# knelk/enerf

Measured on AMD Instinct MI355X. Metric: train_rays_per_sec, higher is better.
Workload: dtype f32

## Files before the change

### enerf_amd/_lib.py

```python
import ctypes
import os

_HERE = os.path.dirname(os.path.abspath(__file__))
LIB_PATH = os.path.join(_HERE, "lib", "libenerf_hip.so")
if os.environ.get("ENERF_LIB_PATH"):
    LIB_PATH = os.environ["ENERF_LIB_PATH"]

_c = ctypes
_vp, _u32, _f32, _int, _sz = _c.c_void_p, _c.c_uint32, _c.c_float, _c.c_int, _c.c_size_t

SIGNATURES = {
    "enerf_near_far_from_aabb": [_vp, _vp, _vp, _u32, _f32, _vp, _vp, _vp],
    "enerf_polar_from_ray": [_vp, _vp, _f32, _u32, _vp, _vp],
    "enerf_morton3D": [_vp, _u32, _vp, _vp],
    "enerf_morton3D_invert": [_vp, _u32, _vp, _vp],
    "enerf_packbits": [_vp, _u32, _f32, _vp, _vp],
    "enerf_march_rays_train": [_vp, _vp, _vp, _f32, _f32, _u32, _u32, _u32, _u32, _u32, _vp, _vp, _vp, _vp, _vp,
                               _vp, _vp, _u32, _vp],
    "enerf_march_fuse_near_far": [_vp, _f32],
    "enerf_march_mirror_count": [_vp],
    "enerf_march_rays_train_ex": [_vp, _vp, _vp, _f32, _f32, _u32, _u32, _u32, _u32, _u32, _vp, _vp, _vp, _vp, _vp,
                                  _vp, _vp, _u32, _u32, _vp],
    "enerf_march_rays_train_count": [_vp, _vp, _vp, _f32, _f32, _u32, _u32, _u32, _u32, _vp, _vp, _vp, _vp, _u32, _u32,
                                     _vp],
# ... 33 lines not shown
    "enerf_grid_encode_backward_ex": [_vp, _vp, _vp, _vp, _vp, _u32, _u32, _u32, _u32, _f32, _u32, _int, _vp, _vp,
                                   _u32, _int, _int, _f32, _f32, _u32, _u32, _vp],
    "enerf_grid_records_discard": [_vp],
    "enerf_mlp32_signal_next_reduce": [_int],
    "enerf_stream_wait_mlp32_signal": [_vp],
    "enerf_debug_workspace_ordering": [_int],
    "enerf_mlp32_valid_rows": [_vp],
    "enerf_mlp32_valid_rows_ex": [_vp, _u32, _u32],
    "enerf_mlp32_io16": [_int],
    "enerf_grid_adam_from_records_ex": [_vp, _vp, _vp, _vp, _vp, _u32, _u32, _f32, _f32, _f32, _f32, _u32, _u32, _vp, _vp,
                                        _vp, _vp, _vp, _vp, _vp, _vp],
    "enerf_grid_adam_from_records": [_vp, _vp, _vp, _vp, _vp, _u32, _u32, _f32, _f32, _f32, _f32, _u32, _vp],
    "enerf_sh_encode_forward": [_vp, _vp, _u32, _u32, _u32, _int, _vp, _int, _vp],
    "enerf_sh_encode_backward": [_vp, _vp, _u32, _u32, _u32, _vp, _vp, _int, _vp],
    "enerf_ffmlp_forward": [_vp, _vp, _u32, _u32, _u32, _u32, _u32, _u32, _u32, _vp, _vp, _int, _vp],
    "enerf_ffmlp_inference": [_vp, _vp, _u32, _u32, _u32, _u32, _u32, _u32, _u32, _vp, _vp, _int, _vp],
    "enerf_ffmlp_backward": [_vp, _vp, _vp, _vp, _u32, _u32, _u32, _u32, _u32, _u32, _u32, _int, _vp, _vp, _vp,
                             _int, _vp],
    "enerf_ffnerf_inference": [_vp, _vp, _vp, _vp, _u32, _int, _vp, _vp, _vp],
    "enerf_mlp32_forward": [_vp, _vp, _u32, _u32, _u32, _u32, _u32, _u32, _vp, _vp, _u32, _u32, _vp, _vp],
    "enerf_mlp32_forward_p": [_vp, _vp, _u32, _u32, _u32, _u32, _u32, _u32, _u32, _u32, _vp, _vp, _u32, _u32, _vp, _vp,
                              _vp],
    "enerf_mlp32_backward_p": [_vp, _vp, _vp, _vp, _u32, _u32, _u32, _vp, _u32, _u32, _u32, _u32, _u32, _vp, _vp, _u32,
                               _u32, _vp, _u32, _vp, _vp, _u32, _vp],
    "enerf_mlp32_forward_sh": [_vp, _vp, _u32, _u32, _u32, _u32, _u32, _u32, _vp, _vp, _u32, _u32, _vp, _vp, _vp],
    "enerf_mlp32_backward": [_vp, _vp, _vp, _vp, _u32, _u32, _u32, _u32, _u32, _vp, _vp, _vp, _u32, _u32, _vp, _u32, _vp, _vp,
                             _u32, _vp],
    "enerf_sh_encode_forward_strided": [_vp, _vp, _u32, _u32, _u32, _vp],
    "enerf_debug_grid_level_mask": [_u32],
    "enerf_debug_sweep_route": [_u32, _u32],
    "enerf_debug_sweep_schedule": [_u32, _u32, _u32, _vp, _u32],
    "enerf_debug_mlp32_wgrad_blocks": [_u32],
    "enerf_debug_mlp32_grid_caps": [_u32, _u32],
    "enerf_debug_march_wave_max_rays": [_u32],
    "enerf_debug_march_bg_blocks": [_u32],
    "enerf_debug_march_clip": [_int],
    "enerf_march_rays_use_box": [_int],
    "enerf_grid_owner_range": [ctypes.c_uint64, ctypes.c_uint64, _f32],
    "enerf_ffmlp_recompute": [_int],
    "enerf_amp_begin": [_vp, _vp, _vp, _vp],
    "enerf_amp_end": [_f32, _f32, _int, _vp],
    "enerf_amp_cancel": [],
    "enerf_debug_march_thread_min_rays": [_u32],
    "enerf_event_loss_fwd_bwd": [_vp, _vp, _vp, _u32, _u32, _u32, _f32, _f32, _f32, _vp, _vp, _vp, _vp, _vp],
    "enerf_event_loss_fwd_bwd_c": [_vp, _vp, _vp, _u32, _u32, _u32, _f32, _f32, _f32, _vp, _vp, _vp, _vp, _u32, _vp],
    "enerf_event_pair_rays": [_vp, _vp, _vp, _vp, _u32, _vp, _vp, _u32, _u32, _vp, _vp, _vp, _vp, _u32, _f32, _f32, _f32,
                              _f32, _vp, _vp, _vp, _vp, _vp, _vp, _vp, _vp, _vp],
    "enerf_event_single_pair_rays": [_vp, _u32, _vp, _vp, _u32, _vp, _vp, _u32, _vp, _vp, _vp, _vp, _u32, _f32, _f32, _f32,
                                     _f32, _vp, _vp, _vp, _vp, _vp, _vp, _vp, _vp, _vp, _vp],
    "enerf_no_event_rays": [_vp, _u32, _vp, _vp, _u32, _c.c_double, _c.c_double, _vp, _vp, _vp, _vp, _u32, _f32, _f32,
                            _f32, _f32, _vp, _vp, _vp, _vp, _vp, _vp, _vp, _vp],
    "enerf_occupied_box_update": [_vp, _u32, _u32, _f32, _vp],
    "enerf_debug_mlp32_fused_backward": [_int],
    "enerf_mlp32_precision": [_int],
    "enerf_mlp32_recompute": [_int],
    "enerf_debug_grid_bwd_binned": [_u32, _u32],
    "enerf_density_grid_cells": [_vp, _u32, _u32, _f32, _u32, _c.c_uint64, _vp, _vp, _vp],
    "enerf_mark_untrained_grid": [_vp, _u32, _u32, _f32, _f32, _f32, _f32, _u32, _u32, _f32, _vp, _vp],
    "enerf_density_grid_update": [_vp, _vp, _u32, _u32, _u32, _f32, _f32, _f32, _vp, _vp, _vp, _u32, _vp, _vp],
    "enerf_adam_step": [_vp, _vp, _vp, _vp, _sz, _f32, _f32, _f32, _f32, _u32, _int, _vp],
    "enerf_allocate_splitk": [_sz],
    "enerf_free_splitk": [],
    "enerf_mlp32_defer_reduce": [_int],
    "enerf_march_train_samples": [_c.POINTER(_c.c_uint64), _int, _vp],
    "enerf_prof_enable": [_int],
    "enerf_prof_reset": [],
# ... 207 lines not shown
```

### enerf_amd/csrc/mlp32.hip

```cpp
#include <hip/hip_runtime.h>
#include <cstdlib>
#include <cstring>
#include <hip/hip_ext.h>

#include "common.h"
#include "mlp32_common.h"
#include "sh_basis.h"

using namespace enerf;
using namespace enerf_mlp32;

namespace {


#ifdef ENERF_MLP_TIMING
__device__ unsigned long long g_mlp_phase[16];
#define MLP_PH(k)                                                  \
    do {                                                           \
        const unsigned long long t_ = __builtin_amdgcn_s_memtime(); \
        ph[k] += t_ - t_last;                                      \
        t_last = t_;                                               \
    } while (0)
#else
#define MLP_PH(k)
// ... 736 lines not shown
}

__global__ void __launch_bounds__(1024) k_mlp32_reduce_w2(ReduceJob a, ReduceJob b, uint32_t* found_inf) {
    const uint32_t na = (a.NW + 63u) / 64u;
    if (blockIdx.x < na) reduce_w_body(a.partial, a.nblocks, a.NW, a.dst, blockIdx.x, found_inf, a.stride);
    else reduce_w_body(b.partial, b.nblocks, b.NW, b.dst, blockIdx.x - na, found_inf, b.stride);
}

static ValidRows g_valid = {nullptr, 0, 0};
static bool g_signal_armed = false;
static bool g_signal_recorded = false;
static hipEvent_t g_signal_event = nullptr;
#ifndef ENERF_SIGNAL_SYSTEM_RELEASE
constexpr unsigned kSignalEventFlags = hipEventDisableTiming | hipEventReleaseToDevice;
#else
constexpr unsigned kSignalEventFlags = hipEventDisableTiming;
#endif
hipEvent_t signal_event() {
    if (!g_signal_event && hipEventCreateWithFlags(&g_signal_event, kSignalEventFlags) != hipSuccess) g_signal_event = nullptr;
    return g_signal_event;
}
static bool g_defer_next = false;
static DeferredReduce g_pending = {};

bool g_fused_bwd = true;
int g_precision = 1;
inline bool ops16(int mode) { return mode == 2 || mode == 3; }
bool g_io16_p = false;
bool g_recompute = true;
inline bool recompute_for(uint32_t num_hidden) { return g_recompute || num_hidden == 3; }
uint32_t g_wgrad_blocks = 0;

uint32_t g_fwd_blocks = 0;
uint32_t g_bwd_blocks = 0;

bool split_bwd_shape(int mode, uint32_t num_hidden, uint32_t out_dim, uint32_t x_layout) {
    return g_fused_bwd && mode != 0 && out_dim <= 16 &&
           (num_hidden <= 2 || (ops16(mode) && num_hidden == 3 && x_layout == 0));
}

uint32_t pgrid(uint32_t B, uint32_t cap) {
    const uint32_t blocks = div_up(div_up(B, 32), 4);
    return blocks < cap ? blocks : cap;
}

}

extern "C" {

int enerf_mlp32_valid_rows(const int32_t* device_count) { return enerf_mlp32_valid_rows_ex(device_count, 0, 0); }
int enerf_mlp32_valid_rows_ex(const int32_t* device_count, uint32_t base, uint32_t cap) {
    g_valid = {device_count, device_count ? base : 0, device_count ? cap : 0};
    return 0;
}

int enerf_mlp32_io16(int on) {
    const int prev = g_io16_p ? 1 : 0;
    if (on >= 0) g_io16_p = on != 0;
    return prev;
}

int enerf_mlp32_precision(int mode) {
    const int prev = g_precision;
    if (mode >= 0 && mode <= 3) g_precision = mode;
    return prev;
}

int enerf_mlp32_recompute(int on) {
    const int prev = g_recompute ? 1 : 0;
    if (on >= 0) g_recompute = on != 0;
    return prev;
}

int enerf_debug_mlp32_fused_backward(int on) {
    g_fused_bwd = on != 0;
    return 0;
}

int enerf_debug_mlp32_grid_caps(uint32_t fwd_blocks, uint32_t bwd_blocks) {
    g_fwd_blocks = fwd_blocks;
    g_bwd_blocks = bwd_blocks;
    return 0;
}

int enerf_debug_mlp32_wgrad_blocks(uint32_t blocks) {
    g_wgrad_blocks = blocks;
    return 0;
}

}


static WSrc seg_src(const float* const* wseg, uint32_t num_hidden, uint32_t w0_cols, uint32_t nerf_perm, const ValidRows& rows) {
    WSrc w;
    for (uint32_t k = 0; k < 4; k++) w.seg[k] = (k == 0 || k == 3 || k < num_hidden) ? wseg[k] : nullptr;
    w.w0_cols = w0_cols;
    w.nerf_perm = nerf_perm;
    w.valid_rows = rows.count;
    w.valid_base = rows.base;
    w.valid_cap = rows.cap;
    return w;
}
static WDst seg_dst(float* const* dwseg, uint32_t num_hidden, uint32_t w0_cols, uint32_t nerf_perm, uint32_t overwrite) {
    WDst d;
    for (uint32_t k = 0; k < 4; k++) d.seg[k] = (k == 0 || k == 3 || k < num_hidden) ? dwseg[k] : nullptr;
    d.w0_cols = w0_cols;
    d.nerf_perm = nerf_perm;
    d.overwrite = overwrite;
    return d;
}
static WSrc blob_src(const float* W, uint32_t num_hidden, const ValidRows& rows) {
    const float* seg[4] = {W, W + HID * IN, W + HID * IN + HID * HID, W + HID * IN + (num_hidden - 1) * HID * HID};
    return seg_src(seg, num_hidden, IN, 0, rows);
}
static WDst blob_dst(float* dW, uint32_t num_hidden, uint32_t overwrite) {
// ... 6 lines not shown
        return ENERF_E_BADARG;
    }
    if ((nerf_perm && w0_cols != 31 && w0_cols != IN) || (!nerf_perm && w0_cols != IN)) {
        set_error("%s: first-layer rows are 32 floats, or 31 / 32 with the NeRF colour permutation", what);
        return ENERF_E_BADARG;
    }
    return 0;
}

static int mlp32_forward_impl(const float* X, WSrc W, uint32_t B, uint32_t in_dim, uint32_t out_dim,
                              uint32_t num_hidden, uint32_t activation, uint32_t output_activation, float* fb, float* Y,
                              uint32_t x_layout, uint32_t y_stride, float* y0_exp, const float* sh_dirs,
                              enerf_stream_t stream, int mode, bool io16) {
    if (B == 0) return 0;
    if (sh_dirs && !((num_hidden == 1 || (num_hidden == 2 && mode != 0)) && x_layout == 1 && Y && out_dim <= 16 &&
                     (y_stride == 0 ? out_dim : y_stride) >= 32))
        ENERF_BADARG("mlp32_forward_sh: needs one hidden layer (two in the bf16 modes), level-major input, out_dim <= 16 "
                     "and rows of >= 32 floats");
    if (in_dim != IN) ENERF_BADARG("mlp32: in_dim must be 32 (pad the input), got %u", in_dim);
    if (out_dim == 0 || out_dim > 32) ENERF_BADARG("mlp32: out_dim must be in [1, 32], got %u", out_dim);
    if (num_hidden < 1 || num_hidden > 3) ENERF_BADARG("mlp32: num_hidden must be 1..3, got %u", num_hidden);
    if (activation != 0 && activation != 6) ENERF_BADARG("mlp32: activation must be relu (0) or none (6)");
    if (x_layout > 1) ENERF_BADARG("mlp32: x_layout must be 0 (row-major) or 1 (level-major), got %u", x_layout);
    if (output_activation != 0 && output_activation != 3 && output_activation != 6)
        ENERF_BADARG("mlp32: output activation must be relu (0), sigmoid (3) or none (6)");
    if (y_stride == 0) y_stride = out_dim;
    if (y_stride < out_dim) ENERF_BADARG("mlp32: y_stride %u < out_dim %u", y_stride, out_dim);
    if (int eg = single_device_guard("mlp32_forward")) return eg;
    hipStream_t s = (hipStream_t)stream;
    ProfScope prof(ENERF_K_FFMLP_FWD, s, mode != 0);
    prof.units((double)B);
    const bool sigma_only_shape = num_hidden == 1 && !fb && !Y && y0_exp && x_layout == 1;
    const bool lds_operands = mode == 1 && !sigma_only_shape;
    const uint32_t grid = pgrid(B, g_fwd_blocks ? g_fwd_blocks : (lds_operands ? 768 : 512));
    size_t lds = sizeof(float) * (HID * IN + (num_hidden - 1) * HID * HID + out_dim * HID);
    if (lds_operands && lds < (size_t)(8 + 8 * (num_hidden - 1)) * 2048) lds = (size_t)(8 + 8 * (num_hidden - 1)) * 2048;
#define MLP32_FWD2(NHV, TR, XLV) \
    k_mlp32_fwd<NHV, TR, XLV><<<grid, 256, lds, s>>>(X, W, fb, Y, B, out_dim, activation, output_activation, y_stride, y0_exp)
#define MLP32_FWD(NHV)                                        \
    do {                                                      \
        if (fb) {                                             \
            if (x_layout == 0) MLP32_FWD2(NHV, true, 0);      \
            else MLP32_FWD2(NHV, true, 1);                    \
        } else {                                              \
            if (x_layout == 0) MLP32_FWD2(NHV, false, 0);     \
            else MLP32_FWD2(NHV, false, 1);                   \
        }                                                     \
    } while (0)
    const bool sigma_only = num_hidden == 1 && !fb && !Y && y0_exp && x_layout == 1;
    if (mode != 0) {
        const bool store_fb = fb != nullptr && !(recompute_for(num_hidden) && split_bwd_shape(mode, num_hidden, out_dim, x_layout));
        (mode == 3 ? mlp32s_f16_launch_fwd : mlp32s_launch_fwd)(
            mode == 1 ? 3 : 1, num_hidden, store_fb, x_layout, sigma_only, X, W, fb, Y, B, out_dim, activation,
            output_activation, y_stride, y0_exp, sh_dirs, grid, lds, s, prof.start(), prof.stop(), io16);
    } else if (sh_dirs) {
        const ShNorm4 nrm = make_sh_norm4();
        if (fb)
            k_mlp32_fwd<1, true, 1, false, true><<<grid, 256, lds, s>>>(X, W, fb, Y, B, out_dim, activation,
                                                                        output_activation, y_stride, y0_exp, sh_dirs, nrm);
        else
            k_mlp32_fwd<1, false, 1, false, true><<<grid, 256, lds, s>>>(X, W, fb, Y, B, out_dim, activation,
                                                                         output_activation, y_stride, y0_exp, sh_dirs, nrm);
    } else if (sigma_only)
        k_mlp32_fwd<1, false, 1, true><<<grid, 256, lds, s>>>(X, W, fb, Y, B, out_dim, activation, output_activation,
                                                              y_stride, y0_exp);
    else if (num_hidden == 1) MLP32_FWD(1);
    else if (num_hidden == 2) MLP32_FWD(2);
    else MLP32_FWD(3);
#undef MLP32_FWD
#undef MLP32_FWD2
    ENERF_LAUNCH_CHECK("mlp32_forward");
    return 0;
}

int enerf::mlp32_forward_p(const float* X, const float* const* wseg, uint32_t w0_cols, uint32_t nerf_perm, uint32_t B,
                           uint32_t in_dim, uint32_t out_dim, uint32_t num_hidden, uint32_t activation,
                           uint32_t output_activation, float* fb, float* Y, uint32_t x_layout, uint32_t y_stride,
                           float* y0_exp, const float* sh_dirs, enerf_stream_t stream, const MlpCall& c) {
    if (num_hidden < 1 || num_hidden > 3) ENERF_BADARG("mlp32: num_hidden must be 1..3, got %u", num_hidden);
    if (int e = segs_ok((const void* const*)wseg, num_hidden, w0_cols, nerf_perm, "mlp32_forward_p")) return e;
    if (c.io16 && c.mode != 3) ENERF_BADARG("mlp32_forward_p: 16-bit I/O (enerf_mlp32_io16) serves precision 3 only");
    if (c.io16 && (num_hidden < 2 || out_dim > 16 || x_layout != 0 || sh_dirs || y0_exp || !Y))
        ENERF_BADARG("mlp32_forward_p: 16-bit I/O needs two or three hidden layers, out_dim <= 16, row-major X, an output "
                     "Y and no SH / density epilogue");
    return mlp32_forward_impl(X, seg_src(wseg, num_hidden, w0_cols, nerf_perm, c.rows), B, in_dim, out_dim, num_hidden,
                              activation, output_activation, fb, Y, x_layout, y_stride, y0_exp, sh_dirs, stream, c.mode, c.io16);
}

static int mlp32_backward_impl(const float* dY, const float* X, WSrc W, const float* fb, uint32_t B, uint32_t in_dim,
                               uint32_t out_dim, uint32_t num_hidden, uint32_t activation, float* bb, float* dX,
                               WDst dW, uint32_t x_layout, uint32_t dy_stride, const float* y_sigmoid,
                               uint32_t y_sigmoid_stride, const float* dsigma, const float* h0, uint32_t h0_stride,
                               enerf_stream_t stream, int mode, bool io16, bool signal, hipEvent_t* signalled,
                               DeferredReduce* pair) {
    if (B == 0) return 0;
    if (in_dim != IN) ENERF_BADARG("mlp32: in_dim must be 32, got %u", in_dim);
// ... 482 lines not shown
```

### enerf_amd/csrc/mlp32_common.h

```cpp
#pragma once
#include <hip/hip_runtime.h>

#include "common.h"
#include "sh_basis.h"

namespace enerf_mlp32 {
using namespace enerf;

typedef float f32x16 __attribute__((ext_vector_type(16)));
constexpr int HID = 64;
constexpr int IN = 32;

__device__ __forceinline__ f32x16 mma(float a, float b, f32x16 c) {
    return __builtin_amdgcn_mfma_f32_32x32x2f32(a, b, c, 0, 0, 0);
}
__device__ __forceinline__ int nrow(int q, int h) { return (q & 3) + 8 * (q >> 2) + 4 * h; }

__device__ __forceinline__ float act_fwd(float x, uint32_t a) { return a == 0 ? (x > 0 ? x : 0.0f) : x; }
__device__ __forceinline__ float out_act_fwd(float x, uint32_t a) {
    return a == 0 ? (x > 0 ? x : 0.0f) : (a == 3 ? 1.0f / (1.0f + expf(-x)) : x);
}

struct DySource {
    const float* dY;
// ... 157 lines not shown
__device__ __forceinline__ float fb_at(const float* tilebase, int srow, int n) {
    return tilebase[(n >> 5) * 1024 + ((n >> 3) & 3) * 256 + (srow + 32 * ((n >> 2) & 1)) * 4 + (n & 3)];
}

template <int XL>
__device__ __forceinline__ int kmap(int p, int h) {
    return XL == 0 ? 16 * h + p : 4 * (p >> 1) + 2 * h + (p & 1);
}

template <int XL>
__device__ __forceinline__ void load_x(const float* __restrict__ X, uint32_t tile, int j, int h, uint32_t B, uint32_t Bp,
                                       float (&x)[16]) {
    const size_t s = (size_t)tile * 32 + j;
    const bool valid = s < B;
    if (XL == 0) {
        const size_t sc = valid ? s : (size_t)B - 1;
#pragma unroll
        for (int v = 0; v < 4; v++) {
            const float4 t = *reinterpret_cast<const float4*>(X + sc * IN + 16 * h + 4 * v);
            x[4 * v] = t.x; x[4 * v + 1] = t.y; x[4 * v + 2] = t.z; x[4 * v + 3] = t.w;
        }
    } else {
#pragma unroll
        for (int q = 0; q < 8; q++) {
            const float2 t = *reinterpret_cast<const float2*>(X + ((size_t)(2 * q + h) * Bp + s) * 2);
            x[2 * q] = t.x; x[2 * q + 1] = t.y;
        }
    }
    if (!valid) {
#pragma unroll
        for (int p = 0; p < 16; p++) x[p] = 0.0f;
    }
}

void mlp32s_launch_fwd(int prec, uint32_t num_hidden, bool train, uint32_t x_layout, bool sigma_only, const float* X, const WSrc& W,
                       float* fb, float* Y, uint32_t B, uint32_t out_dim, uint32_t act, uint32_t out_act,
                       uint32_t y_stride, float* y0_exp, const float* sh_dirs, uint32_t grid, size_t lds, hipStream_t s,
                       hipEvent_t ev_start = nullptr, hipEvent_t ev_stop = nullptr, bool io16 = false);
void mlp32s_launch_bwd(int prec, uint32_t num_hidden, uint32_t x_layout, const DySource& dys, const float* X, const WSrc& W,
                       const float* fb, float* dX, float* partial, uint32_t B, uint32_t out_dim, uint32_t act,
                       uint32_t grid, hipStream_t s, hipEvent_t ev_start = nullptr, hipEvent_t ev_stop = nullptr,
                       bool recompute = false, bool io16 = false);

void mlp32s_f16_launch_fwd(int prec, uint32_t num_hidden, bool train, uint32_t x_layout, bool sigma_only, const float* X,
                           const WSrc& W, float* fb, float* Y, uint32_t B, uint32_t out_dim, uint32_t act, uint32_t out_act,
                           uint32_t y_stride, float* y0_exp, const float* sh_dirs, uint32_t grid, size_t lds, hipStream_t s,
                           hipEvent_t ev_start = nullptr, hipEvent_t ev_stop = nullptr, bool io16 = false);
void mlp32s_f16_launch_bwd(int prec, uint32_t num_hidden, uint32_t x_layout, const DySource& dys, const float* X,
                           const WSrc& W, const float* fb, float* dX, float* partial, uint32_t B, uint32_t out_dim,
                           uint32_t act, uint32_t grid, hipStream_t s, hipEvent_t ev_start = nullptr,
                           hipEvent_t ev_stop = nullptr, bool recompute = false, bool io16 = false);

constexpr uint32_t kNerfFragBytes = 44 * 2048;
constexpr uint32_t kNerfMapBytes = 44 * 512 * 4;
constexpr uint32_t kNerfPartMapBytes = ((HID * IN + 16 * HID) + (HID * IN + HID * HID + 16 * HID)) * 4;
constexpr uint32_t kNerfWsBytes = kNerfFragBytes + kNerfMapBytes + kNerfPartMapBytes;
constexpr uint32_t kNerfPartialStride = (HID * IN + 16 * HID) + (HID * IN + HID * HID + 16 * HID);
constexpr uint32_t kNerfSigmaWords = HID * IN + 16 * HID;
#ifndef NERF_FWD_ONE_PER_CU
constexpr uint32_t kNerfFwdPerCu = 3;
#else
constexpr uint32_t kNerfFwdPerCu = 1;
#endif
void nerf_launch_frags(const float* ws0, const float* ws1, const float* wc0, const float* wc1, const float* wc2,
                       uint32_t w0_cols, uint32_t out_c, uint32_t* frags, hipStream_t s);
void nerf_launch_frag_map(uint32_t w0_cols, uint32_t out_c, uint32_t* map, hipStream_t s);
void nerf_launch_fwd(const float* X, const float* dirs, const uint32_t* frags, float* sigma, float* rgb, uint32_t B,
                     uint32_t out_c, const int32_t* valid_rows, uint32_t valid_base, uint32_t valid_cap, uint32_t grid,
                     hipStream_t s, hipEvent_t ev_start = nullptr, hipEvent_t ev_stop = nullptr);
void nerf_launch_bwd(const float* X, const float* dirs, const float* g_rgb, const float* rgb, const float* g_sigma,
                     float sigma_scale, const uint32_t* frags, float* dX, float* partial, uint32_t B, uint32_t out_c,
                     const int32_t* valid_rows, uint32_t valid_base, uint32_t valid_cap, uint32_t grid, hipStream_t s,
                     hipEvent_t ev_start = nullptr, hipEvent_t ev_stop = nullptr);

int ffmlp16_forward(int dtype, const void* X, const float* W32, uint32_t B, uint32_t num_hidden, uint32_t activation,
                    void* Y, hipStream_t s);
int ffmlp16_backward(int dtype, const void* dY, const void* X, const float* W32, uint32_t B, uint32_t num_hidden,
// ... 4 lines not shown
```

### enerf_amd/csrc/mlp32s.hip

```cpp
#include <hip/hip_runtime.h>
#include <hip/hip_ext.h>

#include "mlp32_common.h"
#include "mlp32s_ops.h"

namespace enerf_mlp32 {


__device__ __forceinline__ void load_x16(const void* __restrict__ X, uint32_t tile, int j, int h, uint32_t B, bf16x8 (&f)[2]) {
    const size_t s = (size_t)tile * 32 + j;
    const bool valid = s < B;
    const size_t sc = valid ? s : (size_t)B - 1;
    const uint4* p = reinterpret_cast<const uint4*>(reinterpret_cast<const elem16*>(X) + sc * IN + 16 * h);
    uint4 a = p[0], b = p[1];
    if (!valid) a = b = make_uint4(0u, 0u, 0u, 0u);
    f[0] = __builtin_bit_cast(bf16x8, a);
    f[1] = __builtin_bit_cast(bf16x8, b);
}
__device__ __forceinline__ void store4_16(void* base, size_t elem, float a, float b, float c, float d) {
    typedef elem16 e4 __attribute__((ext_vector_type(4)));
    const e4 v = {(elem16)a, (elem16)b, (elem16)c, (elem16)d};
    *reinterpret_cast<e4*>(reinterpret_cast<elem16*>(base) + elem) = v;
}

constexpr bool fwd_weights_in_lds(bool SIG, int P) { return P == 3 && !SIG; }
typedef unsigned u32x4w __attribute__((ext_vector_type(4)));

#ifdef ENERF_MLP32S_F16
#define k_mlp32s_fwd k_mlp32h_fwd
#define k_mlp32s_bwd k_mlp32h_bwd
#define k_mlp32s_mark k_mlp32h_mark
#endif
template <int NH, bool TRAIN, int XL, bool SIG = false, bool SH = false, int P = 3, bool IO16 = false>
__global__ void __launch_bounds__(256, fwd_weights_in_lds(SIG, P) ? 3 : 1) k_mlp32s_fwd(const float* __restrict__ X, WSrc W,
                                                    float* __restrict__ fb, float* __restrict__ Y, uint32_t B,
                                                    uint32_t out_dim, uint32_t act, uint32_t out_act, uint32_t y_stride,
                                                    float* __restrict__ y0_exp, const float* __restrict__ sh_dirs = nullptr,
                                                    ShNorm4 nrm = ShNorm4{}) {
    extern __shared__ __attribute__((aligned(16))) float wl[];
    const int lane = lane_id(), j = lane & 31, h = lane >> 5;
    const uint32_t Bp = (B + 31u) & ~31u;
    static_assert(!IO16 || (P == 1 && XL == 0 && !SIG && !SH && !TRAIN), "16-bit I/O: bf16 / fp16 operands, row-major, plain");
    float x[16];
    bf16x8 xraw[2];
    {
        const uint32_t tile0 = blockIdx.x * (blockDim.x >> 6) + (threadIdx.x >> 6);
        if (tile0 < Bp / 32) {
            if constexpr (IO16) load_x16(X, tile0, j, h, B, xraw);
            else load_x<XL>(X, tile0, j, h, B, Bp, x);
        }
    }
    stage_rot(wl, W, NH, out_dim);

    typedef FragT<P> Frag;
    constexpr bool WL = fwd_weights_in_lds(SIG, P);
    Frag w0[2][2], wh[NH > 1 ? NH - 1 : 1][2][2][2], wo[2][2];
    float wsig[2][16];
#pragma unroll
    for (int ob = 0; ob < 2; ob++)
#pragma unroll
        for (int t = 0; t < 2; t++) {
            float v[8];
#pragma unroll
            for (int e = 0; e < 8; e++) v[e] = wl[rot(32 * ob + j, kmap<XL>(8 * t + e, h), IN)];
            w0[ob][t] = split8<P>(v);
        }
#pragma unroll
    for (int l = 0; l < NH - 1; l++)
#pragma unroll
        for (int ob = 0; ob < 2; ob++)
#pragma unroll
            for (int ib = 0; ib < 2; ib++)
#pragma unroll
                for (int t = 0; t < 2; t++) {
                    float v[8];
#pragma unroll
                    for (int e = 0; e < 8; e++)
                        v[e] = wl[HID * IN + rot(l * HID + 32 * ob + j, 32 * ib + nrow(8 * t + e, h), HID)];
// ... 35 lines not shown
        __syncthreads();
#pragma unroll
        for (int ob = 0; ob < 2; ob++)
#pragma unroll
            for (int t = 0; t < 2; t++) put(fidx0(ob, t), w0[ob][t]);
#pragma unroll
        for (int l = 0; l < NH - 1; l++)
#pragma unroll
            for (int ob = 0; ob < 2; ob++)
#pragma unroll
                for (int ib = 0; ib < 2; ib++)
#pragma unroll
                    for (int t = 0; t < 2; t++) put(fidxh(l, ob, ib, t), wh[l][ob][ib][t]);
#pragma unroll
        for (int ib = 0; ib < 2; ib++)
#pragma unroll
            for (int t = 0; t < 2; t++) put(fidxo(ib, t), wo[ib][t]);
        __syncthreads();
    }
    auto get = [&](int f) -> Frag {
        Frag w;
        w.hi = __builtin_bit_cast(bf16x8, fr[(2 * f) * 64 + lane]);
        if constexpr (P == 3) w.lo = __builtin_bit_cast(bf16x8, fr[(2 * f + 1) * 64 + lane]);
        return w;
    };
    auto W0 = [&](int ob, int t) -> Frag { return WL ? get(fidx0(ob, t)) : w0[ob][t]; };
    auto WH = [&](int l, int ob, int ib, int t) -> Frag { return WL ? get(fidxh(l, ob, ib, t)) : wh[l][ob][ib][t]; };
    auto WO = [&](int ib, int t) -> Frag { return WL ? get(fidxo(ib, t)) : wo[ib][t]; };

    const int relu_lim = act == 0 ? 0 : (int)0x80000000;
    const uint32_t ntiles = valid_tiles(W, B, Bp / 32);
    const uint32_t gw = blockIdx.x * (blockDim.x >> 6) + (threadIdx.x >> 6);
    const uint32_t nw = gridDim.x * (blockDim.x >> 6);
    for (uint32_t tile = gw; tile < ntiles; tile += nw) {
        const size_t s = (size_t)tile * 32 + j;
        const bool valid = s < B;
        if (WL) asm volatile("" ::: "memory");
        if (!SIG && tile != gw) {
            if constexpr (IO16) load_x16(X, tile, j, h, B, xraw);
            else load_x<XL>(X, tile, j, h, B, Bp, x);
        }
        float dir0 = 0.0f, dir1 = 0.0f, dir2 = 0.0f;
        if (SH && valid) {
            dir0 = sh_dirs[s * 3]; dir1 = sh_dirs[s * 3 + 1]; dir2 = sh_dirs[s * 3 + 2];
        }
        Frag xf[2];
#pragma unroll
        for (int t = 0; t < 2; t++) {
            if constexpr (IO16) {
                xf[t].hi = xraw[t];
            } else {
                float v[8];
#pragma unroll
                for (int e = 0; e < 8; e++) v[e] = x[8 * t + e];
                xf[t] = split8<P>(v);
            }
        }
        if (SIG && tile + nw < ntiles) load_x<XL>(X, tile + nw, j, h, B, Bp, x);
        f32x16 a[2];
        Frag af[2][2];
#pragma unroll
        for (int ob = 0; ob < 2; ob++) {
            a[ob] = (f32x16)(0.0f);
#pragma unroll
            for (int t = 0; t < 2; t++) a[ob] = mmap(W0(ob, t), xf[t], a[ob]);
#pragma unroll
// ... 490 lines not shown
                *p = add ? *p + a[q] : a[q];
            }
        }
    };
    auto flush_all = [&](bool add) {
#pragma unroll
        for (int ob = 0; ob < 2; ob++) flush(aw0[ob], 0, IN, ob, 0, HID, add);
#pragma unroll
        for (int l = 0; l < NH - 1; l++)
#pragma unroll
            for (int ob = 0; ob < 2; ob++)
#pragma unroll
                for (int nb = 0; nb < 2; nb++) flush(awh[l][ob][nb], HID * IN + l * HID * HID, HID, ob, nb, HID, add);
#pragma unroll
        for (int nb = 0; nb < 2; nb++) flush(awo[nb], HID * IN + (NH - 1) * HID * HID, HID, 0, nb, out_dim, add);
    };
    float* dst = partial + (size_t)blockIdx.x * NW;
    if (NRED == 4) {
        flush_all(false);
        __syncthreads();
        for (uint32_t i = threadIdx.x; i < NW; i += blockDim.x)
            dst[i] = ((lds[i] + lds[NW + i]) + lds[2 * NW + i]) + lds[3 * NW + i];
    } else {
        if (wid < 2) flush_all(false);
        __syncthreads();
        if (wid >= 2) flush_all(true);
        __syncthreads();
        for (uint32_t i = threadIdx.x; i < NW; i += blockDim.x) dst[i] = lds[i] + lds[NW + i];
    }
}

__global__ void k_mlp32s_mark() {}

void MLP32S_LAUNCH_FWD(int prec, uint32_t num_hidden, bool train, uint32_t x_layout, bool sigma_only, const float* X,
                       const WSrc& W, float* fb, float* Y, uint32_t B, uint32_t out_dim, uint32_t act, uint32_t out_act,
                       uint32_t y_stride, float* y0_exp, const float* sh_dirs, uint32_t grid, size_t lds, hipStream_t s,
                       hipEvent_t ev_start, hipEvent_t ev_stop, bool io16) {
    if (ev_start) hipExtLaunchKernelGGL(k_mlp32s_mark, dim3(1), dim3(64), 0, s, nullptr, ev_start, 0);
#define S_FWD(NHV, TR, XLV, SIGV, SHV, PV)                                                                                  \
    hipExtLaunchKernelGGL((k_mlp32s_fwd<NHV, TR, XLV, SIGV, SHV, PV>), dim3(grid), dim3(256), lds, s, nullptr, ev_stop, 0, X, W, \
                          fb, Y, B, out_dim, act, out_act, y_stride, y0_exp, sh_dirs, nrm)
#ifdef ENERF_MLP32S_F16
#define S_FWD_P(NHV, TR, XLV, SIGV, SHV) S_FWD(NHV, TR, XLV, SIGV, SHV, 1)
#else
#define S_FWD_P(NHV, TR, XLV, SIGV, SHV)                 \
    do {                                                 \
        if (prec == 3) S_FWD(NHV, TR, XLV, SIGV, SHV, 3); \
        else S_FWD(NHV, TR, XLV, SIGV, SHV, 1);          \
    } while (0)
#endif
#define S_FWD_IO(NHV)                                                                                                       \
    hipExtLaunchKernelGGL((k_mlp32s_fwd<NHV, false, 0, false, false, 1, true>), dim3(grid), dim3(256), lds, s, nullptr, ev_stop, \
                          0, X, W, fb, Y, B, out_dim, act, out_act, y_stride, y0_exp, sh_dirs, nrm)
#define S_FWD_XL(NHV, TR)                                   \
    do {                                                    \
        if (x_layout == 0) S_FWD_P(NHV, TR, 0, false, false); \
        else S_FWD_P(NHV, TR, 1, false, false);             \
    } while (0)
#define S_FWD_TR(NHV)                   \
    do {                                \
        if (train) S_FWD_XL(NHV, true); \
        else S_FWD_XL(NHV, false);      \
    } while (0)
    const ShNorm4 nrm = sh_dirs ? make_sh_norm4() : ShNorm4{};
    if (io16) {
        if (num_hidden == 2) S_FWD_IO(2);
        else S_FWD_IO(3);
    } else if (sh_dirs) {
        if (num_hidden == 1) {
            if (train) S_FWD_P(1, true, 1, false, true);
            else S_FWD_P(1, false, 1, false, true);
        } else {
            if (train) S_FWD_P(2, true, 1, false, true);
            else S_FWD_P(2, false, 1, false, true);
        }
    } else if (sigma_only) {
        S_FWD_P(1, false, 1, true, false);
    } else if (num_hidden == 1) {
        S_FWD_TR(1);
    } else if (num_hidden == 2) {
        S_FWD_TR(2);
    } else {
        S_FWD_TR(3);
    }
#undef S_FWD_TR
#undef S_FWD_IO
#undef S_FWD_XL
#undef S_FWD_P
#undef S_FWD
}

void MLP32S_LAUNCH_BWD(int prec, uint32_t num_hidden, uint32_t x_layout, const DySource& dys, const float* X,
                       const WSrc& W, const float* fb, float* dX, float* partial, uint32_t B, uint32_t out_dim,
                       uint32_t act, uint32_t grid, hipStream_t s, hipEvent_t ev_start, hipEvent_t ev_stop,
                       bool recompute, bool io16) {
    if (ev_start) hipExtLaunchKernelGGL(k_mlp32s_mark, dim3(1), dim3(64), 0, s, nullptr, ev_start, 0);
    if (io16) {
        if (num_hidden == 2)
            hipExtLaunchKernelGGL((k_mlp32s_bwd<2, 0, 1, true, true>), dim3(grid), dim3(256), 0, s, nullptr, ev_stop, 0, dys, X,
                                  W, fb, dX, partial, B, out_dim, act);
        else
            hipExtLaunchKernelGGL((k_mlp32s_bwd<3, 0, 1, true, true>), dim3(grid), dim3(256), 0, s, nullptr, ev_stop, 0, dys, X,
                                  W, fb, dX, partial, B, out_dim, act);
        return;
    }
#define S_BWD(NHV, XLV, PV, RCV)                                                                                         \
    hipExtLaunchKernelGGL((k_mlp32s_bwd<NHV, XLV, PV, RCV>), dim3(grid), dim3(256), 0, s, nullptr, ev_stop, 0, dys, X, W, fb, \
                          dX, partial, B, out_dim, act)
#define S_BWD_R(NHV, XLV, PV)                     \
    do {                                          \
// ... 28 lines not shown
```

### include/enerf_hip.h

```cpp
#ifndef ENERF_HIP_H
#define ENERF_HIP_H

#include <stddef.h>
#include <stdint.h>

#ifdef __cplusplus
extern "C" {
#endif

typedef void* enerf_stream_t;

#define ENERF_OK 0
#define ENERF_E_BADARG (-1)
#define ENERF_E_NOMEM (-2)
#define ENERF_E_UNSUPPORTED (-3)

#define ENERF_F32 0
#define ENERF_F16 1
#define ENERF_BF16 2

const char* enerf_last_error(void);
#define ENERF_ABI_VERSION 13
int enerf_abi_version(void);
uint64_t enerf_workspace_generation(void);
// ... 223 lines not shown
                            uint32_t B, uint32_t out_c, float* dfeat, uint32_t flags, enerf_stream_t stream);

int enerf_mlp32_forward_sh(const float* X, const float* W, uint32_t B, uint32_t in_dim, uint32_t out_dim,
                           uint32_t num_hidden, uint32_t activation, uint32_t output_activation, float* fb, float* Y,
                           uint32_t x_layout, uint32_t y_stride, float* y0_exp, const float* sh_dirs,
                           enerf_stream_t stream);

int enerf_mlp32_backward(const float* dY, const float* X, const float* W, const float* fb, uint32_t B, uint32_t in_dim,
                         uint32_t out_dim, uint32_t num_hidden, uint32_t activation, float* bb, float* dX, float* dW,
                         uint32_t x_layout, uint32_t dy_stride, const float* y_sigmoid, uint32_t y_sigmoid_stride,
                         const float* dsigma, const float* h0, uint32_t h0_stride, enerf_stream_t stream);

int enerf_mlp32_valid_rows(const int32_t* device_count);
int enerf_mlp32_valid_rows_ex(const int32_t* device_count, uint32_t base, uint32_t cap);
int enerf_mlp32_io16(int on);
int enerf_mlp32_precision(int mode);
int enerf_mlp32_recompute(int on);
int enerf_debug_mlp32_fused_backward(int on);
int enerf_mlp32_defer_reduce(int on);
int enerf_mlp32_signal_next_reduce(int on);
int enerf_stream_wait_mlp32_signal(enerf_stream_t stream);
int enerf_amp_begin(float* scale, int32_t* growth_tracker, uint32_t* found_inf, uint32_t* skipped);
int enerf_amp_end(float growth_factor, float backoff_factor, int32_t growth_interval, enerf_stream_t stream);
int enerf_amp_cancel(void);
int enerf_amp_armed(void);
int enerf_debug_mlp32_wgrad_blocks(uint32_t blocks);
int enerf_debug_march_wave_max_rays(uint32_t n);
int enerf_debug_march_clip(int on);
int enerf_march_rays_use_box(int on);
int enerf_debug_march_thread_min_rays(uint32_t n);
int enerf_debug_workspace_ordering(int on);
int enerf_debug_march_bg_blocks(uint32_t n);
int enerf_debug_mlp32_grid_caps(uint32_t fwd_blocks, uint32_t bwd_blocks);

int enerf_event_pair_rays(const float* events, const uint8_t* no_successor, const int64_t* num_successor,
                          const double* pol_cumsum, uint32_t N, const int64_t* start_draw, const double* u_end,
                          uint32_t M, uint32_t acc_max_num_evs, const double* knots, const double* rot,
                          const double* rotvec, const double* tcoef, uint32_t K, float fx, float fy, float cx, float cy,
                          float* rays_o1, float* rays_d1, float* rays_o2, float* rays_d2, float* pols,
                          int64_t* start_out, int64_t* end_out, int32_t* outside_track, enerf_stream_t stream);

int enerf_event_single_pair_rays(const float* events, uint32_t N, const int64_t* num_at_xy, const int64_t* first_at_xy,
                                 uint32_t P, const double* u_xy, const int64_t* choice, uint32_t M, const double* knots,
                                 const double* rot, const double* rotvec, const double* tcoef, uint32_t K, float fx,
                                 float fy, float cx, float cy, float* rays_o1, float* rays_d1, float* rays_o2,
                                 float* rays_d2, float* pols, int64_t* start_out, int64_t* end_out,
                                 int32_t* outside_track, int32_t* bad_choice, enerf_stream_t stream);
int enerf_no_event_rays(const float* coords, uint32_t n_coords, const int64_t* idx, const double* u, uint32_t n,
                        double t0_us, double t1_us, const double* knots, const double* rot, const double* rotvec,
                        const double* tcoef, uint32_t K, float fx, float fy, float cx, float cy, float* rays_o1,
                        float* rays_d1, float* rays_o2, float* rays_d2, double* tss_out, int32_t* outside_track,
                        int32_t* bad_index, enerf_stream_t stream);

int enerf_event_loss_fwd_bwd(const float* image1, const float* image2, const float* pols, uint32_t N, uint32_t use_luma,
                             uint32_t linlog, float C_thres, float log_thres, float upstream, float* grad_image1,
                             float* grad_image2, float* delta, float* loss, enerf_stream_t stream);

int enerf_event_loss_fwd_bwd_c(const float* image1, const float* image2, const float* pols, uint32_t N, uint32_t use_luma,
                               uint32_t linlog, float C_thres, float log_thres, float upstream, float* grad_image1,
                               float* grad_image2, float* delta, float* loss, uint32_t channels, enerf_stream_t stream);

int enerf_adam_step(float* p, float* g, float* m, float* v, size_t n, float lr, float beta1, float beta2, float eps,
                    uint32_t step, int zero_grad, enerf_stream_t stream);
int enerf_adam_step_multi(uint32_t count, float* const* p, float* const* g, float* const* m, float* const* v,
                          const size_t* n, const float* lr, const uint32_t* step, float beta1, float beta2, float eps,
                          int zero_grad, enerf_stream_t stream);
// ... 201 lines not shown
```

Before: 12.20 million.

## Software-pipeline input loads in the density-only MLP head kernel

Adds a pipelined form of the sigma-only forward kernel. Each wave keeps D=2 tiles of input in flight, issuing the next tile's load before computing the current one, with optional nontemporal loads. Launch bounds move to 2 waves per SIMD and the grid is capped at waves times CUs. The aim is to hide global load latency in this memory-bound head, at the cost of more registers per thread and more complex tail handling.

Result: faster. 12.32 million (median of 6 runs) (+1.0%).

```diff
diff --git a/enerf_amd/_lib.py b/enerf_amd/_lib.py
--- a/enerf_amd/_lib.py
+++ b/enerf_amd/_lib.py
@@ -89,6 +89,7 @@
     "enerf_debug_sweep_schedule": [_u32, _u32, _u32, _vp, _u32],
     "enerf_debug_mlp32_wgrad_blocks": [_u32],
     "enerf_debug_mlp32_grid_caps": [_u32, _u32],
+    "enerf_debug_sigma_head": [_int],
     "enerf_debug_march_wave_max_rays": [_u32],
     "enerf_debug_march_bg_blocks": [_u32],
     "enerf_debug_march_clip": [_int],
diff --git a/enerf_amd/csrc/mlp32.hip b/enerf_amd/csrc/mlp32.hip
--- a/enerf_amd/csrc/mlp32.hip
+++ b/enerf_amd/csrc/mlp32.hip
@@ -792,6 +792,14 @@
 uint32_t g_wgrad_blocks = 0;
 
 uint32_t g_fwd_blocks = 0;
+int g_sig_form = kSigPipelined;
+uint32_t sig_grid_cap(int form) {
+    if (form == kSigOneAhead) return 512u;
+#ifdef ENERF_SIG_HEAD_LAB
+    if (form >= 1000) return (uint32_t)(form / 10 % 10) * num_cus();
+#endif
+    return (uint32_t)kSigWaves * num_cus();
+}
 uint32_t g_bwd_blocks = 0;
 
 bool split_bwd_shape(int mode, uint32_t num_hidden, uint32_t out_dim, uint32_t x_layout) {
@@ -841,6 +849,15 @@
     g_fwd_blocks = fwd_blocks;
     g_bwd_blocks = bwd_blocks;
     return 0;
+}
+
+int enerf_debug_sigma_head(int form) {
+    const int prev = g_sig_form;
+    if (form == kSigOneAhead || form == kSigPipelined) g_sig_form = form;
+#ifdef ENERF_SIG_HEAD_LAB
+    if (form >= 1000) g_sig_form = form;
+#endif
+    return prev;
 }
 
 int enerf_debug_mlp32_wgrad_blocks(uint32_t blocks) {
@@ -913,7 +930,9 @@
     prof.units((double)B);
     const bool sigma_only_shape = num_hidden == 1 && !fb && !Y && y0_exp && x_layout == 1;
     const bool lds_operands = mode == 1 && !sigma_only_shape;
-    const uint32_t grid = pgrid(B, g_fwd_blocks ? g_fwd_blocks : (lds_operands ? 768 : 512));
+    const int sig_form = !sigma_only_shape ? kSigOff : (mode == 0 ? kSigOneAhead : g_sig_form);
+    const uint32_t grid =
+        pgrid(B, g_fwd_blocks ? g_fwd_blocks : (sigma_only_shape ? sig_grid_cap(sig_form) : (lds_operands ? 768 : 512)));
     size_t lds = sizeof(float) * (HID * IN + (num_hidden - 1) * HID * HID + out_dim * HID);
     if (lds_operands && lds < (size_t)(8 + 8 * (num_hidden - 1)) * 2048) lds = (size_t)(8 + 8 * (num_hidden - 1)) * 2048;
 #define MLP32_FWD2(NHV, TR, XLV) \
@@ -928,11 +947,10 @@
             else MLP32_FWD2(NHV, false, 1);                   \
         }                                                     \
     } while (0)
-    const bool sigma_only = num_hidden == 1 && !fb && !Y && y0_exp && x_layout == 1;
     if (mode != 0) {
         const bool store_fb = fb != nullptr && !(recompute_for(num_hidden) && split_bwd_shape(mode, num_hidden, out_dim, x_layout));
         (mode == 3 ? mlp32s_f16_launch_fwd : mlp32s_launch_fwd)(
-            mode == 1 ? 3 : 1, num_hidden, store_fb, x_layout, sigma_only, X, W, fb, Y, B, out_dim, activation,
+            mode == 1 ? 3 : 1, num_hidden, store_fb, x_layout, sig_form, X, W, fb, Y, B, out_dim, activation,
             output_activation, y_stride, y0_exp, sh_dirs, grid, lds, s, prof.start(), prof.stop(), io16);
     } else if (sh_dirs) {
         const ShNorm4 nrm = make_sh_norm4();
@@ -942,7 +960,7 @@
         else
             k_mlp32_fwd<1, false, 1, false, true><<<grid, 256, lds, s>>>(X, W, fb, Y, B, out_dim, activation,
                                                                          output_activation, y_stride, y0_exp, sh_dirs, nrm);
-    } else if (sigma_only)
+    } else if (sigma_only_shape)
         k_mlp32_fwd<1, false, 1, true><<<grid, 256, lds, s>>>(X, W, fb, Y, B, out_dim, activation, output_activation,
                                                               y_stride, y0_exp);
     else if (num_hidden == 1) MLP32_FWD(1);
diff --git a/enerf_amd/csrc/mlp32_common.h b/enerf_amd/csrc/mlp32_common.h
--- a/enerf_amd/csrc/mlp32_common.h
+++ b/enerf_amd/csrc/mlp32_common.h
@@ -213,8 +213,28 @@
         for (int p = 0; p < 16; p++) x[p] = 0.0f;
     }
 }
-
-void mlp32s_launch_fwd(int prec, uint32_t num_hidden, bool train, uint32_t x_layout, bool sigma_only, const float* X, const WSrc& W,
+template <bool NT>
+__device__ __forceinline__ void request_x_lm(const float* __restrict__ X, uint32_t tile, int j, int h, uint32_t Bp,
+                                             float (&x)[16]) {
+    typedef float v2f __attribute__((ext_vector_type(2)));
+    const size_t s = (size_t)tile * 32 + j;
+#pragma unroll
+    for (int q = 0; q < 8; q++) {
+        const v2f* p = reinterpret_cast<const v2f*>(X + ((size_t)(2 * q + h) * Bp + s) * 2);
+        const v2f t = NT ? __builtin_nontemporal_load(p) : *p;
+        x[2 * q] = t.x; x[2 * q + 1] = t.y;
+    }
+}
+__device__ __forceinline__ void zero_rows_past(bool valid, float (&x)[16]) {
+#pragma unroll
+    for (int p = 0; p < 16; p++) x[p] = valid ? x[p] : 0.0f;
+}
+
+constexpr int kSigOff = -1, kSigOneAhead = 0, kSigPipelined = 1;
+constexpr int kSigDepth = 2, kSigWaves = 2;
+constexpr bool kSigNT = true;
+
+void mlp32s_launch_fwd(int prec, uint32_t num_hidden, bool train, uint32_t x_layout, int sig_form, const float* X, const WSrc& W,
                        float* fb, float* Y, uint32_t B, uint32_t out_dim, uint32_t act, uint32_t out_act,
                        uint32_t y_stride, float* y0_exp, const float* sh_dirs, uint32_t grid, size_t lds, hipStream_t s,
                        hipEvent_t ev_start = nullptr, hipEvent_t ev_stop = nullptr, bool io16 = false);
@@ -223,7 +243,7 @@
                        uint32_t grid, hipStream_t s, hipEvent_t ev_start = nullptr, hipEvent_t ev_stop = nullptr,
                        bool recompute = false, bool io16 = false);
 
-void mlp32s_f16_launch_fwd(int prec, uint32_t num_hidden, bool train, uint32_t x_layout, bool sigma_only, const float* X,
+void mlp32s_f16_launch_fwd(int prec, uint32_t num_hidden, bool train, uint32_t x_layout, int sig_form, const float* X,
                            const WSrc& W, float* fb, float* Y, uint32_t B, uint32_t out_dim, uint32_t act, uint32_t out_act,
                            uint32_t y_stride, float* y0_exp, const float* sh_dirs, uint32_t grid, size_t lds, hipStream_t s,
                            hipEvent_t ev_start = nullptr, hipEvent_t ev_stop = nullptr, bool io16 = false);
diff --git a/enerf_amd/csrc/mlp32s.hip b/enerf_amd/csrc/mlp32s.hip
--- a/enerf_amd/csrc/mlp32s.hip
+++ b/enerf_amd/csrc/mlp32s.hip
@@ -1,5 +1,7 @@
 #include <hip/hip_runtime.h>
 #include <hip/hip_ext.h>
+
+#include <type_traits>
 
 #include "mlp32_common.h"
 #include "mlp32s_ops.h"
@@ -31,8 +33,9 @@
 #define k_mlp32s_bwd k_mlp32h_bwd
 #define k_mlp32s_mark k_mlp32h_mark
 #endif
-template <int NH, bool TRAIN, int XL, bool SIG = false, bool SH = false, int P = 3, bool IO16 = false>
-__global__ void __launch_bounds__(256, fwd_weights_in_lds(SIG, P) ? 3 : 1) k_mlp32s_fwd(const float* __restrict__ X, WSrc W,
+template <int NH, bool TRAIN, int XL, bool SIG = false, bool SH = false, int P = 3, bool IO16 = false, int D = 0, int WPS = 1,
+          bool NT = false>
+__global__ void __launch_bounds__(256, fwd_weights_in_lds(SIG, P) ? 3 : WPS) k_mlp32s_fwd(const float* __restrict__ X, WSrc W,
                                                     float* __restrict__ fb, float* __restrict__ Y, uint32_t B,
                                                     uint32_t out_dim, uint32_t act, uint32_t out_act, uint32_t y_stride,
                                                     float* __restrict__ y0_exp, const float* __restrict__ sh_dirs = nullptr,
@@ -41,9 +44,19 @@
     const int lane = lane_id(), j = lane & 31, h = lane >> 5;
     const uint32_t Bp = (B + 31u) & ~31u;
     static_assert(!IO16 || (P == 1 && XL == 0 && !SIG && !SH && !TRAIN), "16-bit I/O: bf16 / fp16 operands, row-major, plain");
-    float x[16];
+    static_assert(D >= 0 && ((SIG && XL == 1 && NH == 1) || (D == 0 && WPS == 1 && !NT)),
+                  "the load pipeline is the density-only head's");
+    constexpr bool PIPE = D > 0;
+    float xq[PIPE ? D : 1][16];
+    float (&x)[16] = xq[0];
     bf16x8 xraw[2];
-    {
+    if constexpr (PIPE) {
+        const uint32_t tile0 = blockIdx.x * (blockDim.x >> 6) + (threadIdx.x >> 6);
+        const uint32_t nw0 = gridDim.x * (blockDim.x >> 6);
+#pragma unroll
+        for (int d = 0; d < D; d++)
+            if (tile0 + (uint32_t)d * nw0 < Bp / 32) request_x_lm<NT>(X, tile0 + (uint32_t)d * nw0, j, h, Bp, xq[d]);
+    } else {
         const uint32_t tile0 = blockIdx.x * (blockDim.x >> 6) + (threadIdx.x >> 6);
         if (tile0 < Bp / 32) {
             if constexpr (IO16) load_x16(X, tile0, j, h, B, xraw);
@@ -145,6 +158,52 @@
     const uint32_t ntiles = valid_tiles(W, B, Bp / 32);
     const uint32_t gw = blockIdx.x * (blockDim.x >> 6) + (threadIdx.x >> 6);
     const uint32_t nw = gridDim.x * (blockDim.x >> 6);
+    if constexpr (PIPE) {
+        auto sig_tile = [&](uint32_t tile, float (&xs)[16], auto steady) __attribute__((always_inline)) {
+            constexpr bool STEADY = decltype(steady)::value;
+            const size_t s = (size_t)tile * 32 + j;
+            const bool valid = STEADY || s < B;
+            if (!STEADY) zero_rows_past(valid, xs);
+            Frag xf[2];
+#pragma unroll
+            for (int t = 0; t < 2; t++) {
+                float v[8];
+#pragma unroll
+                for (int e = 0; e < 8; e++) v[e] = xs[8 * t + e];
+                xf[t] = split8<P>(v);
+            }
+            if (STEADY || tile + D * nw < ntiles) request_x_lm<NT>(X, tile + D * nw, j, h, Bp, xs);
+            f32x16 a[2];
+#pragma unroll
+            for (int ob = 0; ob < 2; ob++) {
+                a[ob] = (f32x16)(0.0f);
+#pragma unroll
+                for (int t = 0; t < 2; t++) a[ob] = mmap(w0[ob][t], xf[t], a[ob]);
+#pragma unroll
+                for (int q = 0; q < 16; q++) a[ob][q] = __int_as_float(max(__float_as_int(a[ob][q]), relu_lim));
+            }
+            float p0 = 0.0f, p1 = 0.0f;
+#pragma unroll
+            for (int q = 0; q < 16; q++) {
+                p0 = fmaf(wsig[0][q], a[0][q], p0);
+                p1 = fmaf(wsig[1][q], a[1][q], p1);
+            }
+            float p = p0 + p1;
+            p += __shfl_xor(p, 32, 64);
+            if (STEADY || (valid && h == 0)) y0_exp[s] = expf(p);
+        };
+        uint32_t tile0 = gw;
+        for (; tile0 + (2 * D - 1) * nw < ntiles; tile0 += D * nw)
+#pragma unroll
+            for (int d = 0; d < D; d++) sig_tile(tile0 + (uint32_t)d * nw, xq[d], std::true_type{});
+        for (; tile0 < ntiles; tile0 += D * nw)
+#pragma unroll
+            for (int d = 0; d < D; d++) {
+                if (d > 0 && tile0 + (uint32_t)d * nw >= ntiles) break;
+                sig_tile(tile0 + (uint32_t)d * nw, xq[d], std::false_type{});
+            }
+        return;
+    }
     for (uint32_t tile = gw; tile < ntiles; tile += nw) {
         const size_t s = (size_t)tile * 32 + j;
         const bool valid = s < B;
@@ -701,7 +760,7 @@
 
 __global__ void k_mlp32s_mark() {}
 
-void MLP32S_LAUNCH_FWD(int prec, uint32_t num_hidden, bool train, uint32_t x_layout, bool sigma_only, const float* X,
+void MLP32S_LAUNCH_FWD(int prec, uint32_t num_hidden, bool train, uint32_t x_layout, int sig_form, const float* X,
                        const WSrc& W, float* fb, float* Y, uint32_t B, uint32_t out_dim, uint32_t act, uint32_t out_act,
                        uint32_t y_stride, float* y0_exp, const float* sh_dirs, uint32_t grid, size_t lds, hipStream_t s,
                        hipEvent_t ev_start, hipEvent_t ev_stop, bool io16) {
@@ -743,8 +802,44 @@
             if (train) S_FWD_P(2, true, 1, false, true);
             else S_FWD_P(2, false, 1, false, true);
         }
-    } else if (sigma_only) {
-        S_FWD_P(1, false, 1, true, false);
+    } else if (sig_form != kSigOff) {
+#define S_SIG(PV, DV, WV, NTV)                                                                                              \
+    hipExtLaunchKernelGGL((k_mlp32s_fwd<1, false, 1, true, false, PV, false, DV, WV, NTV>), dim3(grid), dim3(256), lds, s,   \
+                          nullptr, ev_stop, 0, X, W, fb, Y, B, out_dim, act, out_act, y_stride, y0_exp, sh_dirs, nrm)
+#ifdef ENERF_MLP32S_F16
+#define S_SIG_P(DV, WV, NTV) S_SIG(1, DV, WV, NTV)
+#else
+#define S_SIG_P(DV, WV, NTV)                    \
+    do {                                        \
+        if (prec == 3) S_SIG(3, DV, WV, NTV);   \
+        else S_SIG(1, DV, WV, NTV);             \
+    } while (0)
+#endif
+        if (sig_form == kSigOneAhead) S_SIG_P(0, 1, false);
+#if defined(ENERF_SIG_HEAD_LAB) && !defined(ENERF_MLP32S_F16)
+#define S_SIG_LAB_D(WV, NTV)                                                \
+    do {                                                                    \
+        const int dv = sig_form % 10;                                       \
+        if (dv == 1) S_SIG(3, 1, WV, NTV);                                  \
+        else if (dv == 2) S_SIG(3, 2, WV, NTV);                             \
+        else if (dv == 3) S_SIG(3, 3, WV, NTV);                             \
+        else S_SIG(3, 4, WV, NTV);                                          \
+    } while (0)
+        else if (sig_form >= 1000 && prec == 3) {
+            const bool two = sig_form / 10 % 10 == 2;
+            if (sig_form / 100 % 10) {
+                if (two) S_SIG_LAB_D(2, true);
+                else S_SIG_LAB_D(1, true);
+            } else {
+                if (two) S_SIG_LAB_D(2, false);
+                else S_SIG_LAB_D(1, false);
+            }
+        }
+#undef S_SIG_LAB_D
+#endif
+        else S_SIG_P(kSigDepth, kSigWaves, kSigNT);
+#undef S_SIG_P
+#undef S_SIG
     } else if (num_hidden == 1) {
         S_FWD_TR(1);
     } else if (num_hidden == 2) {
diff --git a/include/enerf_hip.h b/include/enerf_hip.h
--- a/include/enerf_hip.h
+++ b/include/enerf_hip.h
@@ -279,6 +279,7 @@
 int enerf_debug_workspace_ordering(int on);
 int enerf_debug_march_bg_blocks(uint32_t n);
 int enerf_debug_mlp32_grid_caps(uint32_t fwd_blocks, uint32_t bwd_blocks);
+int enerf_debug_sigma_head(int form);
 
 int enerf_event_pair_rays(const float* events, const uint8_t* no_successor, const int64_t* num_successor,
                           const double* pol_cumsum, uint32_t N, const int64_t* start_draw, const double* u_end,
```
